# ViTAE-Transformer/MTP

Measured on AMD Instinct MI355X. Metric: images/sec pretrain step (ViT-L+RVSA, 224^2, bf16), higher is better.
Workload: dtype bf16; 1 GPU; ViT-L + RVSA backbone fwd+bwd + grad all-reduce + clip + AdamW, 224x224, batch 64 per GPU (BASELINE configs[2]/[3]); global_batch=64, parallelism=dp1, activation_checkpointing=False, heads=sum_i mean(f_i)

## Files before the change

### mtp_amd/csrc/gemm.hip

```cpp
#include "gemm_common.h"

namespace {

constexpr int BM = 128;
constexpr int BN = 128;
constexpr int NT_THREADS = 256;
constexpr int ROW_BYTES = 128;
constexpr int OPER_BYTES = BM * ROW_BYTES;
constexpr int STAGE_BYTES = 2 * OPER_BYTES;
constexpr int LDS_BYTES = 2 * STAGE_BYTES;

__device__ __forceinline__ int lds_off(int row, int chunk) { return row * ROW_BYTES + ((chunk ^ (row & 7)) << 4); }

__global__ __launch_bounds__(256) void sum_partials_kernel(const float* __restrict__ part, float* __restrict__ out, int64_t n4, int split) {
    for (int64_t i = (int64_t)blockIdx.x * 256 + threadIdx.x; i < n4; i += (int64_t)gridDim.x * 256) {
        float4 s = *reinterpret_cast<const float4*>(part + 4 * i);
        for (int z = 1; z < split; ++z) {
            const float4 v = *reinterpret_cast<const float4*>(part + 4 * (i + (int64_t)z * n4));
            s.x += v.x; s.y += v.y; s.z += v.z; s.w += v.w;
        }
        *reinterpret_cast<float4*>(out + 4 * i) = s;
    }
}

// ... 414 lines not shown
        }
#pragma unroll
        for (int ni = 0; ni < 4; ++ni)
#pragma unroll
            for (int mi = 0; mi < 4; ++mi) Mma<bf16_t>::run(acc[ni][mi], b[ni], a[mi]);
    }
}

__global__ __launch_bounds__(NT_THREADS) __attribute__((amdgpu_waves_per_eu(4, 4))) void gemm_tn_tr_kernel(KArgs p) {
    extern __shared__ __attribute__((aligned(16))) char smem[];
    const int tid = threadIdx.x, lane = tid & 63, wave = __builtin_amdgcn_readfirstlane(tid >> 6);
    const int wm = wave >> 1, wn = wave & 1;
    const int tile = (p.order & 1) ? (int)blockIdx.x : xcd_remap(blockIdx.x, gridDim.x);
    const int tiles_m = (int)gridDim.x / p.tiles_n;
    const int m0 = ((p.order & 2) ? tile % tiles_m : tile / p.tiles_n) * BM, n0 = ((p.order & 2) ? tile / tiles_m : tile % p.tiles_n) * BN;
    const int kt0 = blockIdx.y * p.k_tiles_per_split;
    int kt1 = kt0 + p.k_tiles_per_split;
    kt1 = kt1 < p.k_tiles ? kt1 : p.k_tiles;
    if (kt0 >= kt1) return;
    p.C += (int64_t)blockIdx.y * p.split_stride * (int64_t)sizeof(float);
    f32x4_t acc[4][4];
#pragma unroll
    for (int i = 0; i < 4; ++i)
#pragma unroll
        for (int j = 0; j < 4; ++j) acc[i][j] = f32x4_t{0.f, 0.f, 0.f, 0.f};
    const bool do_colsum = p.colsum != nullptr && n0 == 0;
    float cs[8] = {0.f, 0.f, 0.f, 0.f, 0.f, 0.f, 0.f, 0.f};
    for (int kt = kt0; kt < kt1; ++kt) {
        stage_tn_glds(p, smem, smem + OPER_BYTES, m0, n0, kt, wave, lane);
        asm volatile("s_waitcnt vmcnt(0)" ::: "memory");
        __syncthreads();
        compute_stage_tr(smem, smem + OPER_BYTES, acc, wm, wn, lane);
        if (do_colsum) {
#pragma unroll
            for (int j = 0; j < 4; ++j) {
                const uint4 v = *reinterpret_cast<const uint4*>(smem + ((tid >> 4) + 16 * j) * TR_ROW_BYTES + (tid & 15) * 16);
                const uint32_t w[4] = {v.x, v.y, v.z, v.w};
#pragma unroll
                for (int e = 0; e < 4; ++e) {
                    cs[2 * e] += __uint_as_float(w[e] << 16);
                    cs[2 * e + 1] += __uint_as_float(w[e] & 0xffff0000u);
                }
            }
        }
        __syncthreads();
    }
    if (do_colsum) {
        float* red = reinterpret_cast<float*>(smem);
        const int rg = tid >> 4, f = (rg & 3) | ((rg >> 1) & 4), chunk = (tid & 15) ^ (f << 1);
        *reinterpret_cast<float4*>(red + rg * BM + chunk * 8) = make_float4(cs[0], cs[1], cs[2], cs[3]);
        *reinterpret_cast<float4*>(red + rg * BM + chunk * 8 + 4) = make_float4(cs[4], cs[5], cs[6], cs[7]);
        __syncthreads();
        if (tid < BM) {
            float s = 0.f;
#pragma unroll
            for (int r = 0; r < 16; ++r) s += red[r * BM + tid];
            if (m0 + tid < p.M) atomicAdd(p.colsum + m0 + tid, s);
        }
    }
    epilogue<float, MTP_EPI_BIAS, 4>(p, acc, m0 + wm * 64, n0 + wn * 64, lane);
}

template <typename T>
int fill_common(const mtp_gemm_args* a, KArgs& k) {
    constexpr int E = Elem<T>::kPerChunk;
    if (!a->A || !a->B || !a->C || a->M <= 0 || a->N <= 0 || a->K <= 0) return MTP_ERR_ARG;
    if (a->M > INT32_MAX || a->N > INT32_MAX || a->K > INT32_MAX) return MTP_ERR_ARG;
    if ((a->lda % E) || (a->ldb % E) || (a->ldc % 4) || (a->N % 4)) return MTP_ERR_ARG;
    if (((uintptr_t)a->A | (uintptr_t)a->B | (uintptr_t)a->C) & 15) return MTP_ERR_ARG;
    k.A = (const char*)a->A; k.B = (const char*)a->B; k.C = (char*)a->C;
    k.M = (int)a->M; k.N = (int)a->N; k.K = (int)a->K;
    k.lda = a->lda; k.ldb = a->ldb; k.ldc = a->ldc;
    k.bias = a->bias; k.bias_mod = (int)a->bias_mod;
    k.res = a->res; k.res_ld = a->res_ld; k.res_mod = (int)a->res_mod;
    k.rowscale = a->rowscale; k.rows_per_sample = (int)(a->rows_per_sample > 0 ? a->rows_per_sample : 1);
    k.aux = (char*)a->aux; k.aux_ld = a->aux_ld;
    k.tiles_n = (int)((a->N + BN - 1) / BN);
    k.k_tiles = (int)((a->K + 8 * E - 1) / (8 * E));
    k.k_tiles_per_split = k.k_tiles;
    k.atomic_out = 0;
    k.order = (a->variant >> 1) & 3;
    k.split_stride = 0;
    k.colsum = nullptr;
    return 0;
}

int nt_p8_mode(const mtp_gemm_args* a, const KArgs& k, int cus) {
    if (a->in_dtype != MTP_BF16 || (a->variant & 1024) || !mtp_nt_p8_fits(k, a->out_dtype, a->epilogue)) return 0;
    const int forced = (a->variant >> 8) & 3;
    if (forced) return forced;
    const int64_t tiles = ((a->M + 255) / 256) * ((a->N + 255) / 256) * 256 / cus;
    return (tiles >= 72 || (tiles >= 40 && a->K >= 1536)) ? 1 : 0;
}

int nt_s8_mode(const mtp_gemm_args* a, const KArgs& k, int cus) {
    if (a->in_dtype != MTP_BF16 || (a->variant & (1024 | (1 << 18))) || ((a->variant >> 8) & 3) || !mtp_nt_s8_fits(k, a->out_dtype, a->epilogue)) return 0;
    if (a->variant & (1 << 17)) return 1;
    const int64_t tiles = ((a->M + 255) / 256) * ((a->N + 255) / 256) * 256 / cus;
    return tiles >= 40 && tiles <= 128;
}

template <typename T, typename Tout, int EPI>
int launch_nt(const mtp_gemm_args* a, hipStream_t stream) {
    constexpr int E = Elem<T>::kPerChunk;
    KArgs k;
    int rc = fill_common<T>(a, k);
    if (rc) return rc;
    if (a->K % E) return MTP_ERR_ARG;
    if (EPI == MTP_EPI_BIAS_RES && (!a->res || (a->res_ld % 4))) return MTP_ERR_ARG;
    if ((EPI == MTP_EPI_BIAS_GELU || EPI == MTP_EPI_DGELU || EPI == MTP_EPI_BIAS_GELU_DG || EPI == MTP_EPI_MUL) && (!a->aux || (a->aux_ld % 4))) return MTP_ERR_ARG;
    if (a->bias && a->bias_mod > 0 && (a->bias_mod % 4)) return MTP_ERR_ARG;
    if constexpr (sizeof(T) == 2) {
        const int cus = mtp_stream_cus(stream);
        if (nt_s8_mode(a, k, cus)) return mtp_nt_s8_launch(k, a->out_dtype, EPI, ((((a->variant >> 1) & 3) == 1) ? 2 : 0), stream);
        const int p8 = nt_p8_mode(a, k, cus);
        if (p8) return mtp_nt_p8_launch(k, a->out_dtype, EPI, (p8 == 2 ? 1 : p8 == 3 ? 4 : 0) | ((((a->variant >> 1) & 3) == 1) ? 2 : 0) | (((a->variant >> 15) & 3) << 8) | (((a->variant >> 20) & 3) << 13), stream);
    }
    const int tiles_m = (k.M + BM - 1) / BM;
    dim3 grid(tiles_m * k.tiles_n), block(NT_THREADS);
    const bool glds = ((a->variant & 1) == 0) && (a->K % (8 * E) == 0);
    const int ord = (a->variant >> 1) & 3;
    k.order = ord == 0 ? (k.tiles_n > 8 ? 2 : 0) : ord == 1 ? 1 : ord == 2 ? 2 : 0;
    if (!glds) k.order = ord;
    const int tiles_m8 = (k.M + NT8_BM - 1) / NT8_BM;
    const bool one_round = tiles_m8 * k.tiles_n >= 256 && tiles_m8 * k.tiles_n <= 512;
    if (glds && ((a->variant & 32) || (one_round && !(a->variant & 64)))) {
        if (ord == 0) k.order = k.tiles_n > 8 ? 2 : 0;
        hipLaunchKernelGGL((gemm_nt_sb8_kernel<T, Tout, EPI>), dim3(tiles_m8 * k.tiles_n), dim3(NT8_THREADS), NT8_STAGE_BYTES, stream, k);
        return mtp_launch_status();
    }
    if (glds)
        hipLaunchKernelGGL((gemm_nt_sb_kernel<T, Tout, EPI>), grid, block, STAGE_BYTES, stream, k);
    else
        hipLaunchKernelGGL((gemm_nt_kernel<T, Tout, EPI, false>), grid, block, LDS_BYTES, stream, k);
    return mtp_launch_status();
}

template <typename T>
int launch_tn(const mtp_gemm_args* a, hipStream_t stream) {
    constexpr int E = Elem<T>::kPerChunk;
    KArgs k;
    int rc = fill_common<T>(a, k);
    if (rc) return rc;
    if (a->out_dtype != MTP_F32 || (a->M % E) || (a->N % E)) return MTP_ERR_ARG;
    k.bias = nullptr;
    int split = a->split_k > 1 ? a->split_k : 1;
    if (split > k.k_tiles) split = k.k_tiles;
    k.k_tiles_per_split = (k.k_tiles + split - 1) / split;
    split = (k.k_tiles + k.k_tiles_per_split - 1) / k.k_tiles_per_split;
    const bool use_ws = split > 1 && a->aux != nullptr;
    k.atomic_out = split > 1 && !use_ws;
    k.split_stride = 0;
    if (split > 1) {
        if (a->ldc != a->N) return MTP_ERR_ARG;
        if (use_ws) {
            if ((uintptr_t)a->aux & 15) return MTP_ERR_ARG;
            k.C = (char*)a->aux;
            k.split_stride = (int64_t)a->M * a->N;
        } else {
            hipError_t e = hipMemsetAsync(a->C, 0, sizeof(float) * (size_t)a->M * (size_t)a->N, stream);
            if (e != hipSuccess) return (int)e;
        }
    }
    const int tiles_m = (k.M + BM - 1) / BM;
    dim3 grid(tiles_m * k.tiles_n, split), block(NT_THREADS);
    const bool full = (a->K % (8 * E) == 0) && (a->M % BM == 0) && (a->N % BN == 0);
    const bool tr = sizeof(T) == 2 && !(a->variant & 16) && (full || ((a->K % 64 == 0) && (a->M % 8 == 0) && (a->N % 8 == 0) && a->M >= 8 && a->N >= 8 && !(a->variant & 32768)));
    if (a->colsum && !tr) {
        rc = mtp_colsum_acc(a->A, a->in_dtype, a->lda, a->colsum, a->K, a->M, stream);
        if (rc) return rc;
    }
    if (tr) {
        k.colsum = a->colsum;
        const int ord = (a->variant >> 1) & 3;
        k.order = ord == 0 ? (a->N > a->M ? 2 : 0) : ord == 1 ? 1 : ord == 2 ? 2 : 0;
        hipLaunchKernelGGL(gemm_tn_tr_kernel, grid, block, STAGE_BYTES, stream, k);
    } else if (full && (a->variant & 8))
        hipLaunchKernelGGL((gemm_tn_sb_kernel<T, true>), grid, block, STAGE_BYTES, stream, k);
    else if (full)
        hipLaunchKernelGGL((gemm_tn_kernel<T, true>), grid, block, LDS_BYTES, stream, k);
    else
        hipLaunchKernelGGL((gemm_tn_kernel<T, false>), grid, block, LDS_BYTES, stream, k);
    if (use_ws && !a->defer_sum) {
        const int64_t n4 = (int64_t)a->M * a->N / 4;
        int64_t nb = (n4 + 255) / 256;
        hipLaunchKernelGGL(sum_partials_kernel, dim3((unsigned)(nb > 4096 ? 4096 : nb)), dim3(256), 0, stream, (const float*)a->aux, (float*)a->C, n4, split);
    }
    return mtp_launch_status();
}

struct SumJobs {
    const float* part[MTP_MAX_SEGMENTS];
    float* out[MTP_MAX_SEGMENTS];
    int64_t n4[MTP_MAX_SEGMENTS];
    int split[MTP_MAX_SEGMENTS];
};
__global__ __launch_bounds__(256) void sum_partials_batch_kernel(SumJobs t) {
    const int j = blockIdx.y;
    const float* __restrict__ part = t.part[j];
// ... 73 lines not shown
```

### mtp_amd/csrc/gemm_common.h

```cpp
#pragma once
#include "common.h"

struct KArgs {
    const char* A;
    const char* B;
    char* C;
    int M, N, K;
    int64_t lda, ldb, ldc;
    const float* bias;
    int bias_mod;
    const float* res;
    int64_t res_ld;
    int res_mod;
    const float* rowscale;
    int rows_per_sample;
    char* aux;
    int64_t aux_ld;
    int tiles_n;
    int k_tiles;
    int k_tiles_per_split;
    int atomic_out;
    int order;
    int64_t split_stride;
    float* colsum;
};

int mtp_nt_p8_launch(const KArgs& k, int out_dtype, int epilogue, int flags, hipStream_t stream);
int mtp_nt_p8_fits(const KArgs& k, int out_dtype, int epilogue);
int mtp_nt_s8_launch(const KArgs& k, int out_dtype, int epilogue, int flags, hipStream_t stream);
int mtp_nt_s8_fits(const KArgs& k, int out_dtype, int epilogue);

namespace {

template <typename T>
struct Mma;
template <>
struct Mma<bf16_t> {
    __device__ static __forceinline__ void run(f32x4_t& acc, const uint4& a, const uint4& b) {
        acc = __builtin_amdgcn_mfma_f32_16x16x32_bf16(__builtin_bit_cast(bf16x8_t, a), __builtin_bit_cast(bf16x8_t, b), acc, 0, 0, 0);
    }
};
template <>
struct Mma<float> {
    __device__ static __forceinline__ void run(f32x4_t& acc, const uint4& a, const uint4& b) {
        acc = __builtin_amdgcn_mfma_f32_16x16x4f32(__uint_as_float(a.x), __uint_as_float(b.x), acc, 0, 0, 0);
        acc = __builtin_amdgcn_mfma_f32_16x16x4f32(__uint_as_float(a.y), __uint_as_float(b.y), acc, 0, 0, 0);
        acc = __builtin_amdgcn_mfma_f32_16x16x4f32(__uint_as_float(a.z), __uint_as_float(b.z), acc, 0, 0, 0);
        acc = __builtin_amdgcn_mfma_f32_16x16x4f32(__uint_as_float(a.w), __uint_as_float(b.w), acc, 0, 0, 0);
    }
};

__device__ __attribute__((aligned(16))) const uint4 g_zero16 = {0u, 0u, 0u, 0u};

__device__ __forceinline__ int xcd_remap(int bid, int nb) {
    int xcd = bid & 7, idx = bid >> 3, q = nb >> 3, r = nb & 7;
    return (xcd < r ? xcd * (q + 1) : r * (q + 1) + (xcd - r) * q) + idx;
}


template <typename Tout, int EPI, int MF>
__device__ __forceinline__ void epilogue(const KArgs& p, f32x4_t (&acc)[4][MF], int mrow0, int ncol0, int lane) {
    const int fr = lane & 15, g = lane >> 4;
    Tout* C = reinterpret_cast<Tout*>(p.C);
    int nn[4];
    bool nok[4];
    float4 bias[4];
#pragma unroll
    for (int ni = 0; ni < 4; ++ni) {
        const int n = ncol0 + ni * 16 + g * 4;
        nok[ni] = n < p.N;
        nn[ni] = nok[ni] ? n : 0;
        const float* bp = (EPI != MTP_EPI_DGELU && EPI != MTP_EPI_MUL && p.bias) ? p.bias + (p.bias_mod > 0 ? nn[ni] % p.bias_mod : nn[ni]) : reinterpret_cast<const float*>(&g_zero16);
        const uint4 b = ldg16(bp);
        bias[ni] = make_float4(__uint_as_float(b.x), __uint_as_float(b.y), __uint_as_float(b.z), __uint_as_float(b.w));
    }
#pragma unroll
    for (int mi = 0; mi < MF; ++mi) {
        const int m = mrow0 + mi * 16 + fr;
        const bool mok = m < p.M;
        const int mc = mok ? m : 0;
        if (p.atomic_out) {
#pragma unroll
            for (int ni = 0; ni < 4; ++ni)
                if (mok && nok[ni]) {
                    float* c = reinterpret_cast<float*>(p.C) + (int64_t)m * p.ldc + nn[ni];
                    atomicAdd(c + 0, acc[ni][mi][0]); atomicAdd(c + 1, acc[ni][mi][1]); atomicAdd(c + 2, acc[ni][mi][2]); atomicAdd(c + 3, acc[ni][mi][3]);
                }
            continue;
        }
        float rs = 1.0f;
        float4 side[4];
        if (EPI == MTP_EPI_BIAS_RES) {
            const float* rsp = p.rowscale ? p.rowscale + mc / p.rows_per_sample : nullptr;
            const float* resrow = p.res + (int64_t)(p.res_mod > 0 ? mc % p.res_mod : mc) * p.res_ld;
#pragma unroll
            for (int ni = 0; ni < 4; ++ni) {
                const uint4 r = ldg16(resrow + nn[ni]);
                side[ni] = make_float4(__uint_as_float(r.x), __uint_as_float(r.y), __uint_as_float(r.z), __uint_as_float(r.w));
            }
            if (rsp) rs = *rsp;
        } else if (EPI == MTP_EPI_DGELU || EPI == MTP_EPI_MUL) {
#pragma unroll
            for (int ni = 0; ni < 4; ++ni) side[ni] = load4(reinterpret_cast<const Tout*>(p.aux) + (int64_t)mc * p.aux_ld + nn[ni]);
        }
#pragma unroll
        for (int ni = 0; ni < 4; ++ni) {
            float4 v = make_float4(acc[ni][mi][0] + bias[ni].x, acc[ni][mi][1] + bias[ni].y, acc[ni][mi][2] + bias[ni].z, acc[ni][mi][3] + bias[ni].w);
// ... 22 lines not shown
```

### mtp_amd/csrc/gemm_p8.hip

```cpp
#include "gemm_p8.h"

namespace {

struct P8Ctx {
    uint32_t addrA[2][2];
    uint32_t addrA1[2][2];
    uint32_t addrB[2][2];
    uint32_t voffA, voffB;
    const char* pA[2][2];
    const char* pB[2][2];
    uint32_t m0base;
};

template <int IMM>
__device__ __forceinline__ void dsr(u32x4_t& d, uint32_t addr) {
    asm volatile("ds_read_b128 %0, %1 offset:%2" : "=v"(d) : "v"(addr), "i"(IMM));
}

template <int SK, int SBUF>
__device__ __forceinline__ void nt_stage(const P8Ctx& c) {
    constexpr int h = (SK == KA1 || SK == KB1) ? 1 : 0;
    const uint32_t l0 = c.m0base + SBUF * P8_BUF + SK * P8_HALF;
    if constexpr (SK == KA0 || SK == KA1)
        glds2(c.voffA, c.pA[h][0], c.pA[h][1], l0, l0 + 1024);
    else
        glds2(c.voffB, c.pB[h][0], c.pB[h][1], l0, l0 + 1024);
}

template <int K, int BUF, int MI>
__device__ __forceinline__ void nt_read_a(const P8Ctx& c, u32x4_t (&a)[2][4]) {
    constexpr int o = K * P8_HALF;
    const uint32_t a0 = K == KA1 ? c.addrA1[BUF][0] : c.addrA[BUF][0], a1 = K == KA1 ? c.addrA1[BUF][1] : c.addrA[BUF][1];
    dsr<o + 0 * 2048>(a[0][0], a0); dsr<o + 1 * 2048>(a[0][1], a0); dsr<o + 2 * 2048>(a[0][2], a0);
    if constexpr (MI == 4) dsr<o + 3 * 2048>(a[0][3], a0);
    dsr<o + 0 * 2048>(a[1][0], a1); dsr<o + 1 * 2048>(a[1][1], a1); dsr<o + 2 * 2048>(a[1][2], a1);
    if constexpr (MI == 4) dsr<o + 3 * 2048>(a[1][3], a1);
}
template <int K, int BUF>
__device__ __forceinline__ void nt_read_b(const P8Ctx& c, u32x4_t (&b)[2][2]) {
    constexpr int o = K * P8_HALF;
    dsr<o + 0 * 2048>(b[0][0], c.addrB[BUF][0]); dsr<o + 1 * 2048>(b[0][1], c.addrB[BUF][0]);
    dsr<o + 0 * 2048>(b[1][0], c.addrB[BUF][1]); dsr<o + 1 * 2048>(b[1][1], c.addrB[BUF][1]);
}
template <int MI>
__device__ __forceinline__ void wait_a(u32x4_t (&a)[2][4]) {
    if constexpr (MI == 4)
        asm volatile("s_waitcnt lgkmcnt(0)"
                     : "+v"(a[0][0]), "+v"(a[0][1]), "+v"(a[0][2]), "+v"(a[0][3]), "+v"(a[1][0]), "+v"(a[1][1]), "+v"(a[1][2]), "+v"(a[1][3]));
    else
        asm volatile("s_waitcnt lgkmcnt(0)" : "+v"(a[0][0]), "+v"(a[0][1]), "+v"(a[0][2]), "+v"(a[1][0]), "+v"(a[1][1]), "+v"(a[1][2]));
}
__device__ __forceinline__ void wait_b(u32x4_t (&b)[2][2]) {
    asm volatile("s_waitcnt lgkmcnt(0)" : "+v"(b[0][0]), "+v"(b[0][1]), "+v"(b[1][0]), "+v"(b[1][1]));
}

template <int MI1>
struct NtOps {
    typedef P8Ctx Ctx;
    static constexpr int kLoadsPerPiecePair = 2;
    static constexpr int kMi1 = MI1;
    template <int K, int BUF> static __device__ __forceinline__ void read_a(Ctx& c, u32x4_t (&a)[2][4]) { nt_read_a<K, BUF, (K == KA1 ? MI1 : 4)>(c, a); }
    template <int K, int BUF> static __device__ __forceinline__ void read_b(Ctx& c, u32x4_t (&b)[2][2]) { nt_read_b<K, BUF>(c, b); }
    template <int SK, int SBUF> static __device__ __forceinline__ void stage(Ctx& c) { nt_stage<SK, SBUF>(c); }
    template <int K, int BUF> static __device__ __forceinline__ void retire_a(Ctx&, u32x4_t (&a)[2][4]) { wait_a<(K == KA1 ? MI1 : 4)>(a); }
    static __device__ __forceinline__ void retire_b(u32x4_t (&b)[2][2]) { wait_b(b); }
    static __device__ __forceinline__ void next_ktile(Ctx& c) { c.voffA += 128; c.voffB += 128; }
};

template <int MI1>
__device__ __forceinline__ void p8_tile_sources(const KArgs& p, P8Ctx& c, int wave, int m0, int n0, uint32_t voffA0, uint32_t voffB0) {
    constexpr int WROWS = 64 + 16 * MI1;
#pragma unroll
    for (int i = 0; i < 2; ++i) {
        const int q = wave * 2 + i;
        int ra0 = m0 + (q >> 3) * WROWS + (q & 7) * 8;
        const int qw = q / (2 * MI1), qx = q - qw * (2 * MI1);
        int ra1 = qw < 2 ? m0 + qw * WROWS + 64 + qx * 8 : m0;
        ra0 = ra0 < p.M - 8 ? ra0 : p.M - 8;
        ra1 = ra1 < p.M - 8 ? ra1 : p.M - 8;
        c.pA[0][i] = p.A + (int64_t)ra0 * p.lda * 2;
        c.pA[1][i] = p.A + (int64_t)ra1 * p.lda * 2;
#pragma unroll
        for (int h = 0; h < 2; ++h) {
            int rb = n0 + (q >> 2) * 64 + h * 32 + (q & 3) * 8;
            rb = rb < p.N - 8 ? rb : p.N - 8;
            c.pB[h][i] = p.B + (int64_t)rb * p.ldb * 2;
        }
    }
    c.voffA = voffA0;
    c.voffB = voffB0;
}
__device__ __forceinline__ void p8_issue_prologue(P8Ctx& c) {
    nt_stage<KB1, 0>(c); nt_stage<KA0, 0>(c); nt_stage<KB0, 0>(c); nt_stage<KA1, 0>(c);
    c.voffA += 128; c.voffB += 128;
    nt_stage<KB0, 1>(c); nt_stage<KA0, 1>(c); nt_stage<KB1, 1>(c); nt_stage<KA1, 1>(c);
    c.voffA += 128; c.voffB += 128;
}

template <typename Tout, int EPI, int MI1, int XP, int PS, int SP = 0>
__global__ __launch_bounds__(P8_THREADS) __attribute__((amdgpu_waves_per_eu(2, 2))) void gemm_nt_p8_kernel(KArgs p) {
    extern __shared__ __attribute__((aligned(16))) char smem[];
    constexpr int WROWS = 64 + 16 * MI1, BM = 2 * WROWS;
    const int tid = threadIdx.x, lane = tid & 63;
    const int wave = __builtin_amdgcn_readfirstlane(tid >> 6);
    const int wr = wave >> 2, wc = wave & 3;
    const int fr = lane & 15, g = lane >> 4;
    const uint32_t lds0 = (uint32_t)(uintptr_t)(__attribute__((address_space(3))) char*)(smem);
    const int tiles_m = (p.M + BM - 1) / BM, tiles_n = p.tiles_n, ntiles = tiles_m * tiles_n;
    const int plain = p.order & 1;
    const int pairs = p.k_tiles >> 1;

    P8Ctx c;
    {
        const uint32_t lanepart = (uint32_t)(fr * 128 + ((g ^ (fr & 7)) << 4));
#pragma unroll
        for (int b = 0; b < 2; ++b) {
            c.addrA[b][0] = lds0 + b * P8_BUF + wr * 8192 + lanepart;
            c.addrA[b][1] = lds0 + b * P8_BUF + wr * 8192 + (lanepart ^ 64u);
            c.addrA1[b][0] = lds0 + b * P8_BUF + wr * (MI1 * 2048) + lanepart;
            c.addrA1[b][1] = lds0 + b * P8_BUF + wr * (MI1 * 2048) + (lanepart ^ 64u);
            c.addrB[b][0] = lds0 + b * P8_BUF + wc * 4096 + lanepart;
            c.addrB[b][1] = lds0 + b * P8_BUF + wc * 4096 + (lanepart ^ 64u);
        }
        c.m0base = lds0 + wave * 2048;
    }
    const uint32_t lanesrc = (uint32_t)(((lane & 7) ^ (lane >> 3)) << 4);
    const uint32_t voffA0 = (uint32_t)((lane >> 3) * (int)p.lda * 2) + lanesrc;
    const uint32_t voffB0 = (uint32_t)((lane >> 3) * (int)p.ldb * 2) + lanesrc;

    int tile = blockIdx.x;
    int tm, tn;
    tile_coords(plain ? tile : xcd_remap(tile, ntiles), tiles_m, tiles_n, plain, tm, tn);
    int m0 = tm * BM, n0 = tn * P8_BN;
    p8_tile_sources<MI1>(p, c, wave, m0, n0, voffA0, voffB0);
    p8_issue_prologue(c);

    u32x4_t a[2][4], b0[2][2], b1[2][2];
    f32x4_t acc[4][8];
    for (;;) {
#pragma unroll
        for (int i = 0; i < 4; ++i)
#pragma unroll
            for (int j = 0; j < 8; ++j) acc[i][j] = f32x4_t{0.f, 0.f, 0.f, 0.f};

        wait_vm<12>();
        __builtin_amdgcn_sched_barrier(0);
        __builtin_amdgcn_s_barrier();
        __builtin_amdgcn_sched_barrier(0);
        nt_read_b<KB1, 0>(c, b1);
        wait_b(b1);
        __builtin_amdgcn_sched_barrier(0);
        __builtin_amdgcn_s_barrier();
        if (!(XP & 2) && wr == 1) __builtin_amdgcn_s_barrier();
        __builtin_amdgcn_sched_barrier(0);

        for (int it = 0; it < pairs - 1; ++it) two_tiles<NtOps<MI1>, false, XP>(c, a, b0, b1, acc);
        two_tiles<NtOps<MI1>, true, XP>(c, a, b0, b1, acc);

        __builtin_amdgcn_sched_barrier(0);
        if (!(XP & 2) && wr == 0) __builtin_amdgcn_s_barrier();
        __builtin_amdgcn_sched_barrier(0);

        if constexpr (PS) {
            const int em0 = m0, en0 = n0;
            tile += gridDim.x;
            const bool more = tile < ntiles;
            if (more) {
                tile_coords(plain ? tile : xcd_remap(tile, ntiles), tiles_m, tiles_n, plain, tm, tn);
                m0 = tm * BM; n0 = tn * P8_BN;
                p8_tile_sources<MI1>(p, c, wave, m0, n0, voffA0, voffB0);
                p8_issue_prologue(c);
            }
            __builtin_amdgcn_sched_barrier(0);
            epilogue_lds16<Tout, EPI, WROWS, SP>(p, acc, smem + P8_LDS + wave * 4096, em0 + wr * WROWS, en0 + wc * 64, lane);
            if (!more) break;
            __builtin_amdgcn_sched_barrier(0);
            wait_vm<0>();
        } else {
            if constexpr (SP != 0) {
                epilogue_lds16<Tout, EPI, WROWS, SP>(p, acc, smem + P8_LDS + wave * 4096, m0 + wr * WROWS, n0 + wc * 64, lane);
            } else if (!(XP & 4) || p.M < 0) {
                if constexpr (XP & 16)
                    epilogue<Tout, EPI, 8>(p, acc, m0 + wr * 128, n0 + wc * 64, lane);
                else
                    epilogue_lds<Tout, EPI, 64, 32, WROWS>(p, acc, smem + wave * P8_HALF, m0 + wr * WROWS, n0 + wc * 64, lane);
            }
            break;
        }
    }
}

template <typename Tout, int EPI, int MI1, int XP, int PS = 0, int SP = 0>
int launch_p8_kernel(const KArgs& a, int ntiles, hipStream_t stream) {
    constexpr int LDS = P8_LDS + ((PS || SP) ? 8 * 4096 : 0);
    static unsigned long long optin = 0;
    if (const int e = mtp_optin_lds((const void*)gemm_nt_p8_kernel<Tout, EPI, MI1, XP, PS, SP>, LDS, optin)) return e;
    const int cus = mtp_stream_cus(stream);
    const int grid = PS ? (ntiles < cus ? ntiles : cus) : ntiles;
    hipLaunchKernelGGL((gemm_nt_p8_kernel<Tout, EPI, MI1, XP, PS, SP>), dim3(grid), dim3(P8_THREADS), LDS, stream, a);
    return mtp_launch_status();
}

int p8_pick_bm(int64_t M, int64_t N, int64_t cus) {
    const int64_t tn = (N + P8_BN - 1) / P8_BN;
    const int64_t t256 = ((M + 255) / 256) * tn, t224 = ((M + 223) / 224) * tn;
    const int64_t c256 = ((t256 + cus - 1) / cus) * 256, c224 = ((t224 + cus - 1) / cus) * 224;
    return c224 < c256 ? 224 : 256;
}

template <typename Tout, int EPI>
int launch_p8(const KArgs& k, int flags, hipStream_t stream) {
    const int bm = (flags & 1) ? 224 : (flags & 4) ? 256 : p8_pick_bm(k.M, k.N, mtp_stream_cus(stream));
    const int tiles_m = (k.M + bm - 1) / bm, tiles_n = (k.N + P8_BN - 1) / P8_BN;
    KArgs a = k;
    a.tiles_n = tiles_n;
    a.k_tiles = k.K / 64;
    a.order = (flags >> 1) & 1;
    a.atomic_out = 0;
    const int ntiles = tiles_m * tiles_n;
    const bool persist = (flags & 256) || (!(flags & 512) && bm == 224 && ntiles > mtp_stream_cus(stream));
    int sp = (flags >> 13) & 3;
    if (sp == 0) sp = (EPI == MTP_EPI_BIAS_RES) ? 2 : 1;
    if (bm == 224 && sp == 1) return persist ? launch_p8_kernel<Tout, EPI, 3, 0, 1, 1>(a, ntiles, stream) : launch_p8_kernel<Tout, EPI, 3, 0, 0, 1>(a, ntiles, stream);
    if (bm == 224 && sp == 2) return persist ? launch_p8_kernel<Tout, EPI, 3, 0, 1, 2>(a, ntiles, stream) : launch_p8_kernel<Tout, EPI, 3, 0, 0, 2>(a, ntiles, stream);
    if (persist) {
        if (bm == 224) return launch_p8_kernel<Tout, EPI, 3, 0, 1>(a, ntiles, stream);
        return launch_p8_kernel<Tout, EPI, 4, 0, 1>(a, ntiles, stream);
    }
    if (bm == 224) return launch_p8_kernel<Tout, EPI, 3, 0>(a, ntiles, stream);
    return launch_p8_kernel<Tout, EPI, 4, 0>(a, ntiles, stream);
}

template <typename Tout>
int dispatch_p8(const KArgs& k, int epi, int flags, hipStream_t s) {
    switch (epi) {
        case MTP_EPI_BIAS: return launch_p8<Tout, MTP_EPI_BIAS>(k, flags, s);
        case MTP_EPI_BIAS_GELU: return launch_p8<Tout, MTP_EPI_BIAS_GELU>(k, flags, s);
        case MTP_EPI_DGELU: return launch_p8<Tout, MTP_EPI_DGELU>(k, flags, s);
        case MTP_EPI_BIAS_GELU_DG: return launch_p8<Tout, MTP_EPI_BIAS_GELU_DG>(k, flags, s);
        case MTP_EPI_MUL: return launch_p8<Tout, MTP_EPI_MUL>(k, flags, s);
        default: return MTP_ERR_UNSUPPORTED;
    }
}

}

int mtp_nt_p8_fits(const KArgs& k, int out_dtype, int epi) {
    if (k.K < 128 || (k.K % 128) || (k.M % 8) || (k.N % 8) || k.M < 8 || k.N < 8) return 0;
    if ((uint64_t)k.lda * 2 * 8 + (uint64_t)k.K * 2 >= (1ull << 31) || (uint64_t)k.ldb * 2 * 8 + (uint64_t)k.K * 2 >= (1ull << 31)) return 0;
    if (epi == MTP_EPI_BIAS_RES) return out_dtype == MTP_F32;
    if (out_dtype == MTP_BF16) return epi == MTP_EPI_BIAS || epi == MTP_EPI_BIAS_GELU || epi == MTP_EPI_DGELU || epi == MTP_EPI_BIAS_GELU_DG || epi == MTP_EPI_MUL;
    return out_dtype == MTP_F32 && epi == MTP_EPI_BIAS;
}

int mtp_nt_p8_launch(const KArgs& k, int out_dtype, int epi, int flags, hipStream_t stream) {
    if (!mtp_nt_p8_fits(k, out_dtype, epi)) return MTP_ERR_UNSUPPORTED;
    if (epi == MTP_EPI_BIAS_RES) return launch_p8<float, MTP_EPI_BIAS_RES>(k, flags, stream);
    if (out_dtype == MTP_BF16) return dispatch_p8<bf16_t>(k, epi, flags, stream);
    return launch_p8<float, MTP_EPI_BIAS>(k, flags, stream);
}
```

### mtp_amd/engine.py

```python
import os

import torch

from . import ops

F32 = torch.float32


class _Blk:
    __slots__ = ("window", "pre", "wqkv", "wqkvT", "wproj", "wprojT", "w1", "w1T", "w2", "w2T", "wsamp", "bsamp", "bproj", "b2", "wproj_s", "w2_s")


class BackboneEngine:
    def __init__(self, module, act_dtype=torch.bfloat16):
        self.m = module
        self.act = act_dtype
        self.C = module.embed_dim
        self.depth = len(module.blocks)
        self.heads = module.num_heads
        self.hd = self.C // self.heads
        self.scale = module.qk_scale if module.qk_scale is not None else self.hd ** -0.5
        self.window = [bool(w) for w in module.window_blocks]
        self.out_indices = list(module.out_indices)
        self._key = None
        self._ln_parts = []
        self._sl_jobs = []
        self._blk = None
        self._fpn = None
        self._pe = None
        self._wimg = None
        self._wimg_ptrs = None
        self._ls = []
        self._zero_rel = {}

    def params(self):
        return dict(self.m.named_parameters())

    def _weights_key(self, P):
        return (self.act,) + tuple((p.data_ptr(), p._version) for p in P.values())

    def prepare_weights(self, force=False):
        P = self.params()
        key = self._weights_key(P)
        if not force and key == self._key:
            return
        ptrs = (self.act,) + tuple(p.data_ptr() for p in P.values())
        if self._wimg is None or ptrs != self._wimg_ptrs:
            self._build_weight_images(P)
            self._wimg_ptrs = ptrs
        with torch.no_grad():
            for pre, b in self._ls:
                g1, g2 = P[pre + "gamma_1"].detach(), P[pre + "gamma_2"].detach()
                torch.mul(P[pre + "attn.proj.weight"].detach(), g1[:, None], out=b.wproj_s)
                torch.mul(P[pre + "mlp.fc2.weight"].detach(), g2[:, None], out=b.w2_s)
                torch.mul(P[pre + "attn.proj.bias"].detach(), g1, out=b.bproj)
                torch.mul(P[pre + "mlp.fc2.bias"].detach(), g2, out=b.b2)
        if force or getattr(self, "_images_fresh", None) != key:
            self._wimg.refresh()
        self._images_fresh = None
        for name, (wg, wgT) in self._fpn.items():
            ops.convt_pack(P[name + ".weight"].detach().contiguous(), wg, wgT)
        self._key = key

    def mark_images_fresh(self):
        self._images_fresh = self._weights_key(self.params())
        self._key = None

    def _build_weight_images(self, P):
        dev = P["patch_embed.proj.weight"].device
        act, H, C = self.act, self.heads, self.C
        entries = []

        def both(w2d):
            w2d = w2d.detach()
            assert w2d.is_contiguous()
            R, Cc = w2d.shape
            wt = torch.empty(Cc, R, device=dev, dtype=act)
            w = w2d if act == F32 else torch.empty(R, Cc, device=dev, dtype=act)
            entries.append((w2d, None if act == F32 else w, wt, False))
            return w, wt

        ls = getattr(self.m, "init_values", None) is not None
        self._ls = []

        blks = []
        for i in range(self.depth):
            b = _Blk()
            b.window = self.window[i]
            b.pre = pre = "blocks.%d." % i
# ... 63 lines not shown
        return ops.colsum(dy, out, accumulate=True)

    def _ln_bwd(self, *args, **kw):
        return ops.layernorm_bwd(*args, accumulate=True, defer=self._ln_parts, **kw)

    def _ln_flush(self):
        if self._ln_parts:
            ops.reduce_rows_deferred(self._ln_parts)
        if self._sl_jobs:
            ops.small_linear_dw_segments_flush(self._sl_jobs)

    def _full_rel(self, pre, Hp, Wp):
        h = self.P.get(pre + "attn.full_attn_rel_pos_h")
        if h is not None:
            w = self.P[pre + "attn.full_attn_rel_pos_w"]
            if h.shape[0] < 2 * Hp - 1 or w.shape[0] < 2 * Wp - 1:
                raise ValueError("%sattn.full_attn_rel_pos_h/w have %d / %d rows, a %d x %d token grid needs %d / %d (resize them like "
                                 "init_weights does, or build the model for this input size)" % (pre, h.shape[0], w.shape[0], Hp, Wp, 2 * Hp - 1, 2 * Wp - 1))
            return h[:2 * Hp - 1], w[:2 * Wp - 1]
        key = (Hp, Wp)
        if self._zero_rel.get(key) is None:
            self._zero_rel[key] = (torch.zeros(2 * Hp - 1, self.hd, device=self.dev, dtype=F32),
                                   torch.zeros(2 * Wp - 1, self.hd, device=self.dev, dtype=F32))
        return self._zero_rel[key]

    def _drop_scales(self, B, training):
        rates = [float(self.m.drop_path_rates[i]) for i in range(self.depth)]
        live = [training and r > 0.0 and self.m.blocks[i].training for i, r in enumerate(rates)]
        if not any(live):
            return [(None, None)] * self.depth
        keep = torch.tensor([1.0 - r for r in rates], dtype=F32).to(self.dev, non_blocking=True).view(self.depth, 1, 1)
        s = torch.floor(keep + torch.rand(self.depth, 2, B, device=self.dev, dtype=F32)) / keep
        return [(s[i, 0], s[i, 1]) if live[i] else (None, None) for i in range(self.depth)]

    def _block_fwd(self, i, x, B, Hp, Wp, dps, save):
        P, b, C, T, N = self.P, self._blk[i], self.C, x.shape[0], Hp * Wp
        pre = b.pre
        s = {}
        mean1, rstd1 = self._e(T, dtype=F32), self._e(T, dtype=F32)
        ln1 = ops.layernorm_fwd(x, P[pre + "norm1.weight"], P[pre + "norm1.bias"], self._e(T, C), mean1, rstd1)
        if b.window:
            nh, nw = ops.rvsa_windows(Hp, Wp)
            R = B * nh * nw
            avg, pooled = self._e(R, C, dtype=F32), self._e(R, C, dtype=F32)
            samp = ops.rvsa_sampling_fwd(ln1, b.wsamp, b.bsamp, avg, pooled, self._e(R, 5 * self.heads, dtype=F32), B, Hp, Wp)
        qkv = ops.gemm_nt(ln1, b.wqkv, self._e(T, 3 * C), bias=P[pre + "attn.qkv.bias"])
        o = self._e(T, C)
        if b.window:
            lse = self._e(R * self.heads * 49, dtype=F32)
            ops.rvsa_attn_fwd(qkv, samp, o, lse, P[pre + "attn.rel_pos_h"], P[pre + "attn.rel_pos_w"],
                              P[pre + "attn.relative_position_bias_table"], B, Hp, Wp, self.heads, self.scale)
            s.update(avg=avg, pooled=pooled, samp=samp)
        else:
            lse = self._e(B * self.heads * N, dtype=F32)
            rel_h, rel_w = self._full_rel(pre, Hp, Wp)
            ops.full_attn_fwd(qkv, o, lse, rel_h, rel_w, B, Hp, Wp, self.heads, self.scale)
        x1 = ops.gemm_nt(o, b.wproj, self._e(T, C, dtype=F32), epi=ops.EPI_BIAS_RES, bias=b.bproj, res=x,
                         rowscale=dps[0], rows_per_sample=N)
        mean2, rstd2 = self._e(T, dtype=F32), self._e(T, dtype=F32)
        ln2 = ops.layernorm_fwd(x1, P[pre + "norm2.weight"], P[pre + "norm2.bias"], self._e(T, C), mean2, rstd2)
        u = self._e(T, 4 * C)
        h = ops.gemm_nt(ln2, b.w1, self._e(T, 4 * C), epi=ops.EPI_BIAS_GELU_DG, bias=P[pre + "mlp.fc1.bias"], aux=u)
        x2 = ops.gemm_nt(h, b.w2, self._e(T, C, dtype=F32), epi=ops.EPI_BIAS_RES, bias=b.b2, res=x1,
                         rowscale=dps[1], rows_per_sample=N)
        if save:
            s.update(x=x, mean1=mean1, rstd1=rstd1, ln1=ln1, qkv=qkv, o=o, lse=lse, x1=x1, mean2=mean2, rstd2=rstd2, ln2=ln2, u=u, h=h)
        return x2, s

    def _layer_scale_grads(self, pre, lin, gname, G):
        P = self.P
        gw, gb, gam = G[pre + lin + ".weight"], G[pre + lin + ".bias"], P[pre + gname]
        G[pre + gname].add_((gw * P[pre + lin + ".weight"]).sum(1) + gb * P[pre + lin + ".bias"])
        gw.mul_(gam[:, None])
        gb.mul_(gam)

    def _block_bwd(self, i, s, dx2, dx2_act, B, Hp, Wp, dps, G, extra, prev_scale):
        P, b, C, N = self.P, self._blk[i], self.C, Hp * Wp
        pre = b.pre
        T = dx2.shape[0]
        wq = self._wq
        ls = pre + "gamma_1" in G
        wq.add(dx2_act, s["h"], G[pre + "mlp.fc2.weight"], G[pre + "mlp.fc2.bias"], after=(lambda: self._layer_scale_grads(pre, "mlp.fc2", "gamma_2", G)) if ls else None,
               norm_ok=not ls)
        du = ops.gemm_nt(dx2_act, b.w2T, self._e(T, 4 * C), epi=ops.EPI_MUL, aux=s["u"])
        wq.add(du, s["ln2"], G[pre + "mlp.fc1.weight"], G[pre + "mlp.fc1.bias"])
        dln2 = ops.gemm_nt(du, b.w1T, self._e(T, C))
        del du
        dx1, dx1_act = self._e(T, C, dtype=F32), self._e(T, C)
        self._ln_bwd(dln2, s["x1"], s["mean2"], s["rstd2"], P[pre + "norm2.weight"], dx1, G[pre + "norm2.weight"], G[pre + "norm2.bias"],
                          dres=dx2, dx_copy=dx1_act, copy_scale=dps[0], rows_per_sample=N)
        wq.add(dx1_act, s["o"], G[pre + "attn.proj.weight"], G[pre + "attn.proj.bias"], after=(lambda: self._layer_scale_grads(pre, "attn.proj", "gamma_1", G)) if ls else None,
               norm_ok=not ls)
        do = ops.gemm_nt(dx1_act, b.wprojT, self._e(T, C))
        dqkv = self._e(T, 3 * C)
        if b.window:
            nh, nw = ops.rvsa_windows(Hp, Wp)
            R = B * nh * nw
            H = self.heads
            dsamp = self._e(R, 5 * H, dtype=F32)
            ops.rvsa_attn_bwd(s["qkv"], s["samp"], s["o"], do, s["lse"], dqkv, dsamp,
                              P[pre + "attn.rel_pos_h"], P[pre + "attn.rel_pos_w"], P[pre + "attn.relative_position_bias_table"],
                              G[pre + "attn.rel_pos_h"], G[pre + "attn.rel_pos_w"], G[pre + "attn.relative_position_bias_table"],
                              B, Hp, Wp, H, self.scale, accumulate=True, defer=self._ln_parts)
            names = ("sampling_offsets", "sampling_scales", "sampling_angles")
            self._sl_jobs.append((s["pooled"], dsamp, [G[pre + "attn.%s.2.weight" % n].view(-1, C) for n in names],
                                  [G[pre + "attn.%s.2.bias" % n] for n in names]))
        else:
            rel_h, rel_w = self._full_rel(pre, Hp, Wp)
            if pre + "attn.full_attn_rel_pos_h" in G:
                drel_h, drel_w = G[pre + "attn.full_attn_rel_pos_h"][:2 * Hp - 1], G[pre + "attn.full_attn_rel_pos_w"][:2 * Wp - 1]
            else:
                drel_h, drel_w = self._e(*rel_h.shape, dtype=F32), self._e(*rel_w.shape, dtype=F32)
            ops.full_attn_bwd(s["qkv"], s["o"], do, s["lse"], dqkv, rel_h, rel_w, drel_h, drel_w, B, Hp, Wp, self.heads, self.scale,
                              accumulate=True, defer=self._ln_parts)
        wq.add(dqkv, s["ln1"], G[pre + "attn.qkv.weight"], G[pre + "attn.qkv.bias"])
        win_add = None
        if b.window:
            win_add = ops.rvsa_sampling_bwd_win(dsamp, b.wsamp, s["avg"], self._e(*s["avg"].shape, dtype=F32))
        dln1 = ops.gemm_nt(dqkv, b.wqkvT, self._e(T, C))
        dx0, dx0_act = self._e(T, C, dtype=F32), self._e(T, C)
        self._ln_bwd(dln1, s["x"], s["mean1"], s["rstd1"], P[pre + "norm1.weight"], dx0, G[pre + "norm1.weight"], G[pre + "norm1.bias"],
                          dres=dx1, extra=extra, dx_copy=dx0_act, copy_scale=prev_scale, rows_per_sample=N,
                          **(dict(win_add=win_add, grid=(B, Hp, Wp)) if win_add is not None else {}))
        return dx0, dx0_act

    def forward(self, img, training=False, need_grad=False, feature_dtype=None):
        m = self.m
        self.dev = img.device
        self.prepare_weights()
        self.P = P = {k: v.detach() for k, v in self.params().items()}
        C, act = self.C, self.act
        ps = m.patch_size
        fdt = feature_dtype or act
        if img.dtype == torch.uint8:
            pp = getattr(m, "data_preprocessor", None)
            if pp is None:
                raise ValueError("uint8 input needs ViT_Win_RVSA_V3_WSZ7.set_data_preprocessor(mean, std, ...)")
            B, H, W, Cin = img.shape
            Hp, Wp = ops.padded_grid(H, W, ps, pp["pad_size_divisor"])
            N, T = Hp * Wp, B * Hp * Wp
            cols = ops.preprocess_patchify(img.contiguous(), self._e(T, Cin * ps * ps), ps, pp["mean"], pp["std"], pp["bgr_to_rgb"],
                                           pp["pad_size_divisor"], pp["pad_value"])
            H, W = Hp * ps, Wp * ps
        else:
            B, Cin, H, W = img.shape
            Hp, Wp = H // ps, W // ps
            N, T = Hp * Wp, B * Hp * Wp
            img = img.contiguous()
            if img.dtype != F32:
                img = img.float()
            cols = ops.patchify(img, self._e(T, Cin * ps * ps), ps)
        pos = P.get("pos_embed")
        if pos is not None:
            assert pos.shape[1] == N, "pos_embed does not match the input size"
            x = ops.gemm_nt(cols, self._pe[0], self._e(T, C, dtype=F32), epi=ops.EPI_BIAS_RES, bias=P["patch_embed.proj.bias"],
                            res=pos.reshape(N, C), res_mod=N)
        else:
            x = ops.gemm_nt(cols, self._pe[0], self._e(T, C, dtype=F32), bias=P["patch_embed.proj.bias"])
        dps = self._drop_scales(B, training)
        ckpt = bool(m.use_checkpoint) and need_grad
        saved, taps = [], {}
        vitdet = bool(getattr(m, "_vitdet", False))
        last = self.depth - 1 if vitdet else max(self.out_indices)
        for i in range(self.depth):
            if i > last:
                break
            xin = x
# ... 10 lines not shown
        else:
            tap_list = [taps[i] for i in self.out_indices]
        if getattr(m, "_taps_only", False):
            feats = [ops.tokens_to_nchw(t, self._e(B, C, Hp, Wp, dtype=fdt), B, Hp, Wp, 0) for t in tap_list]
            fctx = {"taps_only": True}
        else:
            feats, fctx = self._fpn_fwd(tap_list, B, Hp, Wp, fdt, need_grad)
        ctx = None
        if need_grad:
            ctx = dict(saved=saved, dps=dps, fctx=fctx, cols=cols, geom=(B, Cin, H, W, Hp, Wp), ckpt=ckpt, last=last, final=final)
        return feats, ctx

    def _fpn_fwd(self, taps, B, Hp, Wp, fdt, need_grad):
        P, C, T = self.P, self.C, B * Hp * Wp
        m = self.m
        feats, fctx = [], {}
        if m.patch_size == 8:
            t0 = taps[0] if self.act == F32 else ops.cast(taps[0], self._e(T, C))
            z = ops.gemm_nt(t0, self._fpn["fpn1.0"][0], self._e(T, 4 * C), bias=P["fpn1.0.bias"], bias_mod=C)
            feats.append(ops.tokens_to_nchw(z.view(4 * T, C), self._e(B, C, 2 * Hp, 2 * Wp, dtype=fdt), B, Hp, Wp, 1))
            feats.append(ops.tokens_to_nchw(taps[1], self._e(B, C, Hp, Wp, dtype=fdt), B, Hp, Wp, 0))
            H2, W2, H4, W4 = Hp // 2, Wp // 2, Hp // 4, Wp // 4
            p3 = ops.maxpool2_tokens_fwd(taps[2], self._e(B * H2 * W2, C), B, Hp, Wp)
            feats.append(ops.tokens_to_nchw(p3, self._e(B, C, H2, W2, dtype=fdt), B, H2, W2, 0))
            q1 = ops.maxpool2_tokens_fwd(taps[3], self._e(B * H2 * W2, C, dtype=F32), B, Hp, Wp)
            q2 = ops.maxpool2_tokens_fwd(q1, self._e(B * H4 * W4, C), B, H2, W2)
            feats.append(ops.tokens_to_nchw(q2, self._e(B, C, H4, W4, dtype=fdt), B, H4, W4, 0))
            if need_grad:
                fctx = dict(p8=True, t0=t0, tap2=taps[2], tap3=taps[3], q1=q1)
            return feats, fctx
        if m.patch_size != 16:
            raise NotImplementedError("the reference defines the FPN tail for patch_size 16 and 8 only (VIT:640-670)")
        t0 = taps[0] if self.act == F32 else ops.cast(taps[0], self._e(T, C))
        y1 = ops.gemm_nt(t0, self._fpn["fpn1.0"][0], self._e(T, 4 * C), bias=P["fpn1.0.bias"], bias_mod=C)
        mean, rstd = self._e(4 * T, dtype=F32), self._e(4 * T, dtype=F32)
        g1 = ops.layernorm_fwd(y1.view(4 * T, C), P["fpn1.1.ln.weight"], P["fpn1.1.ln.bias"], self._e(4 * T, C), mean, rstd, gelu=True)
        y2 = ops.gemm_nt(g1, self._fpn["fpn1.3"][0], self._e(4 * T, 4 * C), bias=P["fpn1.3.bias"], bias_mod=C)
        feats.append(ops.tokens_to_nchw(y2.view(16 * T, C), self._e(B, C, 4 * Hp, 4 * Wp, dtype=fdt), B, Hp, Wp, 2))
        t1 = taps[1] if self.act == F32 else ops.cast(taps[1], self._e(T, C))
        z = ops.gemm_nt(t1, self._fpn["fpn2.0"][0], self._e(T, 4 * C), bias=P["fpn2.0.bias"], bias_mod=C)
        feats.append(ops.tokens_to_nchw(z.view(4 * T, C), self._e(B, C, 2 * Hp, 2 * Wp, dtype=fdt), B, Hp, Wp, 1))
        feats.append(ops.tokens_to_nchw(taps[2], self._e(B, C, Hp, Wp, dtype=fdt), B, Hp, Wp, 0))
        Ho, Wo = Hp // 2, Wp // 2
        pooled = ops.maxpool2_tokens_fwd(taps[3], self._e(B * Ho * Wo, C), B, Hp, Wp)
        feats.append(ops.tokens_to_nchw(pooled, self._e(B, C, Ho, Wo, dtype=fdt), B, Ho, Wo, 0))
        if need_grad:
            fctx = dict(t0=t0, y1=y1, mean=mean, rstd=rstd, g1=g1, t1=t1, tap3=taps[3])
        return feats, fctx

    def _convt_wgrad(self, dy, x, gw):
        dwg = self._e(dy.shape[1], x.shape[1], dtype=F32)
        self._wq.add(dy, x, dwg, after=lambda: ops.convt_unpack_grad(dwg, gw), norm_of=gw)

    def _fpn_bwd(self, dfeats, fctx, B, Hp, Wp, G):
        P, C, T, act = self.P, self.C, B * Hp * Wp, self.act
        out = [None] * 4

        def as_in(df):
            df = df.contiguous()
            return df if df.dtype in (F32, torch.bfloat16) else df.float()

        if fctx.get("p8"):
            H2, W2, H4, W4 = Hp // 2, Wp // 2, Hp // 4, Wp // 4
            if dfeats[0] is not None:
                dz = ops.nchw_to_tokens(as_in(dfeats[0]), self._e(4 * T, C), B, Hp, Wp, 1)
                self._convt_wgrad(dz.view(T, 4 * C), fctx["t0"], G["fpn1.0.weight"])
                self._colsum(dz, G["fpn1.0.bias"])
                out[0] = ops.gemm_nt(dz.view(T, 4 * C), self._fpn["fpn1.0"][1], self._e(T, C, dtype=F32))
            if dfeats[1] is not None:
                out[1] = ops.nchw_to_tokens(as_in(dfeats[1]), self._e(T, C, dtype=F32), B, Hp, Wp, 0)
            if dfeats[2] is not None:
                dp = ops.nchw_to_tokens(as_in(dfeats[2]), self._e(B * H2 * W2, C, dtype=F32), B, H2, W2, 0)
                out[2] = ops.maxpool2_tokens_bwd(fctx["tap2"], dp, self._e(T, C, dtype=F32), B, Hp, Wp)
            if dfeats[3] is not None:
                dq2 = ops.nchw_to_tokens(as_in(dfeats[3]), self._e(B * H4 * W4, C, dtype=F32), B, H4, W4, 0)
                dq1 = ops.maxpool2_tokens_bwd(fctx["q1"], dq2, self._e(B * H2 * W2, C, dtype=F32), B, H2, W2)
                out[3] = ops.maxpool2_tokens_bwd(fctx["tap3"], dq1, self._e(T, C, dtype=F32), B, Hp, Wp)
            return out

        if dfeats[0] is not None:
            dy2 = ops.nchw_to_tokens(as_in(dfeats[0]), self._e(16 * T, C), B, Hp, Wp, 2)
            self._convt_wgrad(dy2.view(4 * T, 4 * C), fctx["g1"], G["fpn1.3.weight"])
            self._colsum(dy2, G["fpn1.3.bias"])
            dg1 = ops.gemm_nt(dy2.view(4 * T, 4 * C), self._fpn["fpn1.3"][1], self._e(4 * T, C))
            dy1 = self._e(4 * T, C)
            self._ln_bwd(dg1, fctx["y1"].view(4 * T, C), fctx["mean"], fctx["rstd"], P["fpn1.1.ln.weight"], dy1,
                              G["fpn1.1.ln.weight"], G["fpn1.1.ln.bias"], beta=P["fpn1.1.ln.bias"], gelu=True)
            self._convt_wgrad(dy1.view(T, 4 * C), fctx["t0"], G["fpn1.0.weight"])
            self._colsum(dy1, G["fpn1.0.bias"])
            out[0] = ops.gemm_nt(dy1.view(T, 4 * C), self._fpn["fpn1.0"][1], self._e(T, C, dtype=F32))
        if dfeats[1] is not None:
            dz = ops.nchw_to_tokens(as_in(dfeats[1]), self._e(4 * T, C), B, Hp, Wp, 1)
            self._convt_wgrad(dz.view(T, 4 * C), fctx["t1"], G["fpn2.0.weight"])
            self._colsum(dz, G["fpn2.0.bias"])
            out[1] = ops.gemm_nt(dz.view(T, 4 * C), self._fpn["fpn2.0"][1], self._e(T, C, dtype=F32))
        if dfeats[2] is not None:
            out[2] = ops.nchw_to_tokens(as_in(dfeats[2]), self._e(T, C, dtype=F32), B, Hp, Wp, 0)
        if dfeats[3] is not None:
            Ho, Wo = Hp // 2, Wp // 2
            dp = ops.nchw_to_tokens(as_in(dfeats[3]), self._e(B * Ho * Wo, C, dtype=F32), B, Ho, Wo, 0)
            out[3] = ops.maxpool2_tokens_bwd(fctx["tap3"], dp, self._e(T, C, dtype=F32), B, Hp, Wp)
        return out

    def backward(self, ctx, dfeats, G, need_input_grad=False, on_block_done=None, split_last=False, sqn=None):
        B, Cin, H, W, Hp, Wp = ctx["geom"]
        C, N, T = self.C, Hp * Wp, B * Hp * Wp
        P = self.P
        self.dev = ctx["cols"].device
        self._ln_parts = []
        self._sl_jobs = []
        self._wq = wq = ops.WgradQueue(stream=self._wgrad_stream())
        wq.max_jobs = self.wgrad_max_jobs if wq.stream is not None else 0
        wq.sqn = sqn
        self.norm_covered = wq.covered
        if ctx["fctx"].get("taps_only"):
            dtaps = [None if d is None else ops.nchw_to_tokens((d.contiguous() if d.dtype in (F32, torch.bfloat16) else d.float().contiguous()),
                                                               self._e(T, C, dtype=F32), B, Hp, Wp, 0) for d in dfeats]
        else:
            dtaps = self._fpn_bwd(dfeats, ctx["fctx"], B, Hp, Wp, G)
        tapgrad = {}
        last, dps, saved = ctx["last"], ctx["dps"], ctx["saved"]
        if ctx.get("final") is not None:
            dsum = None
            for d in dtaps:
                if d is None:
                    continue
                if dsum is None:
                    dsum = d
                else:
                    ops.axpy(dsum, d)
            if dsum is not None:
                xl, fm, fr = ctx["final"]
                tapgrad[last] = self._ln_bwd(dsum, xl, fm, fr, P["norm.weight"], self._e(T, C, dtype=F32), G["norm.weight"], G["norm.bias"])
        else:
            for idx, d in zip(self.out_indices, dtaps):
                if d is None:
                    continue
                if idx in tapgrad:
                    ops.axpy(tapgrad[idx], d)
                else:
                    tapgrad[idx] = d
        self._ln_flush()
        if on_block_done is not None and not wq.jobs:
            on_block_done(self.depth)
        if last not in tapgrad:
            tapgrad[last] = torch.zeros(T, C, device=self.dev, dtype=F32)
        dx = tapgrad[last]
        dx_act = self._scaled_copy(dx, dps[last][1], N)
        waiting = []
        pending = []
        for i in range(last, -1, -1):
            s = saved[i]
            if ctx["ckpt"]:
                _, s = self._block_fwd(i, s["x"], B, Hp, Wp, dps[i], save=True)
            extra = tapgrad.get(i - 1) if i > 0 else None
            prev_scale = dps[i - 1][1] if i > 0 else None
            dx, dx_act = self._block_bwd(i, s, dx, dx_act, B, Hp, Wp, dps[i], G, extra, prev_scale)
            saved[i] = None
            waiting.append(i)
            if i == 0:
                wq.add(dx_act, ctx["cols"], G["patch_embed.proj.weight"].view(C, -1), G["patch_embed.proj.bias"])
            if i == 0 or wq.should_flush() or not wq.jobs or (split_last and i == 1):
                wq.flush()
                self._ln_flush()
                if wq.stream is None:
                    if on_block_done is not None:
                        on_block_done(waiting[-1])
# ... 24 lines not shown
```

Measured before the change: 1894 images/sec.

## Stagger persistent p8 GEMM blocks and use grouped tile order for tail balance

```diff
diff --git a/mtp_amd/csrc/gemm.hip b/mtp_amd/csrc/gemm.hip
--- a/mtp_amd/csrc/gemm.hip
+++ b/mtp_amd/csrc/gemm.hip
@@ -520,6 +520,8 @@
     k.order = (a->variant >> 1) & 3;
     k.split_stride = 0;
     k.colsum = nullptr;
+    k.stagger_from = 0;
+    k.stagger_ticks = 0;
     return 0;
 }
 
@@ -552,7 +554,7 @@
         const int cus = mtp_stream_cus(stream);
         if (nt_s8_mode(a, k, cus)) return mtp_nt_s8_launch(k, a->out_dtype, EPI, ((((a->variant >> 1) & 3) == 1) ? 2 : 0), stream);
         const int p8 = nt_p8_mode(a, k, cus);
-        if (p8) return mtp_nt_p8_launch(k, a->out_dtype, EPI, (p8 == 2 ? 1 : p8 == 3 ? 4 : 0) | ((((a->variant >> 1) & 3) == 1) ? 2 : 0) | (((a->variant >> 15) & 3) << 8) | (((a->variant >> 20) & 3) << 13), stream);
+        if (p8) return mtp_nt_p8_launch(k, a->out_dtype, EPI, (p8 == 2 ? 1 : p8 == 3 ? 4 : 0) | ((((a->variant >> 1) & 3) == 1) ? 2 : 0) | (((a->variant >> 15) & 3) << 8) | (((a->variant >> 20) & 3) << 13) | (((a->variant >> 22) & 15) << 16), stream);
     }
     const int tiles_m = (k.M + BM - 1) / BM;
     dim3 grid(tiles_m * k.tiles_n), block(NT_THREADS);
diff --git a/mtp_amd/csrc/gemm_common.h b/mtp_amd/csrc/gemm_common.h
--- a/mtp_amd/csrc/gemm_common.h
+++ b/mtp_amd/csrc/gemm_common.h
@@ -23,6 +23,8 @@
     int order;
     int64_t split_stride;
     float* colsum;
+    int stagger_from;
+    int stagger_ticks;
 };
 
 int mtp_nt_p8_launch(const KArgs& k, int out_dtype, int epilogue, int flags, hipStream_t stream);
diff --git a/mtp_amd/csrc/gemm_p8.hip b/mtp_amd/csrc/gemm_p8.hip
--- a/mtp_amd/csrc/gemm_p8.hip
+++ b/mtp_amd/csrc/gemm_p8.hip
@@ -1,3 +1,6 @@
+#include <atomic>
+#include <cstdlib>
+
 #include "gemm_p8.h"
 
 namespace {
@@ -97,6 +100,17 @@
     c.voffA += 128; c.voffB += 128;
 }
 
+__device__ __forceinline__ void p8_coords(int t, int tiles_m, int tiles_n, int order, int& tm, int& tn) {
+    const int per = 8 * tiles_n, grp = t / per, r = t - grp * per;
+    if ((order & 5) == 4 && tiles_m - grp * 8 >= 8 && (tiles_n & 3) == 0) {
+        const int b16 = r >> 4, j = r & 15;
+        tm = grp * 8 + (b16 & 1) * 4 + (j & 3);
+        tn = (b16 >> 1) * 4 + (j >> 2);
+        return;
+    }
+    tile_coords(t, tiles_m, tiles_n, order & 1, tm, tn);
+}
+
 template <typename Tout, int EPI, int MI1, int XP, int PS, int SP = 0>
 __global__ __launch_bounds__(P8_THREADS) __attribute__((amdgpu_waves_per_eu(2, 2))) void gemm_nt_p8_kernel(KArgs p) {
     extern __shared__ __attribute__((aligned(16))) char smem[];
@@ -128,9 +142,15 @@
     const uint32_t voffA0 = (uint32_t)((lane >> 3) * (int)p.lda * 2) + lanesrc;
     const uint32_t voffB0 = (uint32_t)((lane >> 3) * (int)p.ldb * 2) + lanesrc;
 
+    if constexpr (PS) {
+        if (p.stagger_ticks > 0 && (int)blockIdx.x >= p.stagger_from) {
+            const uint64_t until = wall_clock64() + (uint64_t)p.stagger_ticks;
+            while (wall_clock64() < until) __builtin_amdgcn_s_sleep(8);
+        }
+    }
     int tile = blockIdx.x;
     int tm, tn;
-    tile_coords(plain ? tile : xcd_remap(tile, ntiles), tiles_m, tiles_n, plain, tm, tn);
+    p8_coords(plain ? tile : xcd_remap(tile, ntiles), tiles_m, tiles_n, p.order, tm, tn);
     int m0 = tm * BM, n0 = tn * P8_BN;
     p8_tile_sources<MI1>(p, c, wave, m0, n0, voffA0, voffB0);
     p8_issue_prologue(c);
@@ -166,7 +186,7 @@
             tile += gridDim.x;
             const bool more = tile < ntiles;
             if (more) {
-                tile_coords(plain ? tile : xcd_remap(tile, ntiles), tiles_m, tiles_n, plain, tm, tn);
+                p8_coords(plain ? tile : xcd_remap(tile, ntiles), tiles_m, tiles_n, p.order, tm, tn);
                 m0 = tm * BM; n0 = tn * P8_BN;
                 p8_tile_sources<MI1>(p, c, wave, m0, n0, voffA0, voffB0);
                 p8_issue_prologue(c);
@@ -190,6 +210,25 @@
     }
 }
 
+int p8_ticks_per_us() {
+    static std::atomic<int> rate[64];
+    int dev = 0;
+    if (hipGetDevice(&dev) != hipSuccess || dev < 0 || dev >= 64) return 100;
+    int r = rate[dev].load(std::memory_order_relaxed);
+    if (!r) {
+        int khz = 0;
+        if (hipDeviceGetAttribute(&khz, hipDeviceAttributeWallClockRate, dev) != hipSuccess || khz < 1000) khz = 100000;
+        r = khz / 1000;
+        rate[dev].store(r, std::memory_order_relaxed);
+    }
+    return r;
+}
+
+int p8_stagger_env() {
+    static const int v = []() { const char* e = getenv("MTP_NT_STAGGER"); return e && (e[0] == '0' || e[0] == '1') ? e[0] - '0' : -1; }();
+    return v;
+}
+
 template <typename Tout, int EPI, int MI1, int XP, int PS = 0, int SP = 0>
 int launch_p8_kernel(const KArgs& a, int ntiles, hipStream_t stream) {
     constexpr int LDS = P8_LDS + ((PS || SP) ? 8 * 4096 : 0);
@@ -219,6 +258,19 @@
     a.atomic_out = 0;
     const int ntiles = tiles_m * tiles_n;
     const bool persist = (flags & 256) || (!(flags & 512) && bm == 224 && ntiles > mtp_stream_cus(stream));
+    a.stagger_from = 0;
+    a.stagger_ticks = 0;
+    if (persist) {
+        const int cus = mtp_stream_cus(stream), grid = ntiles < cus ? ntiles : cus, rem = ntiles % grid;
+        const int env = p8_stagger_env();
+        const bool on = env >= 0 ? env == 1 : (flags & (1 << 16)) ? true : (flags & (1 << 17)) ? false : true;
+        if (on && rem) {
+            const int q = ((flags >> 18) & 3) ? ((flags >> 18) & 3) : 2;
+            a.stagger_from = rem;
+            a.stagger_ticks = (int)((int64_t)q * a.k_tiles * 1030 * p8_ticks_per_us() / 4000);
+            a.order |= 4;
+        }
+    }
     int sp = (flags >> 13) & 3;
     if (sp == 0) sp = (EPI == MTP_EPI_BIAS_RES) ? 2 : 1;
     if (bm == 224 && sp == 1) return persist ? launch_p8_kernel<Tout, EPI, 3, 0, 1, 1>(a, ntiles, stream) : launch_p8_kernel<Tout, EPI, 3, 0, 0, 1>(a, ntiles, stream);
diff --git a/mtp_amd/engine.py b/mtp_amd/engine.py
--- a/mtp_amd/engine.py
+++ b/mtp_amd/engine.py
@@ -5,6 +5,7 @@
 from . import ops
 
 F32 = torch.float32
+BWD_NT_VARIANT = 0
 
 
 class _Blk:
@@ -234,7 +235,7 @@
         ls = pre + "gamma_1" in G
         wq.add(dx2_act, s["h"], G[pre + "mlp.fc2.weight"], G[pre + "mlp.fc2.bias"], after=(lambda: self._layer_scale_grads(pre, "mlp.fc2", "gamma_2", G)) if ls else None,
                norm_ok=not ls)
-        du = ops.gemm_nt(dx2_act, b.w2T, self._e(T, 4 * C), epi=ops.EPI_MUL, aux=s["u"])
+        du = ops.gemm_nt(dx2_act, b.w2T, self._e(T, 4 * C), epi=ops.EPI_MUL, aux=s["u"], variant=BWD_NT_VARIANT)
         wq.add(du, s["ln2"], G[pre + "mlp.fc1.weight"], G[pre + "mlp.fc1.bias"])
         dln2 = ops.gemm_nt(du, b.w1T, self._e(T, C))
         del du
@@ -411,7 +412,7 @@
             dy2 = ops.nchw_to_tokens(as_in(dfeats[0]), self._e(16 * T, C), B, Hp, Wp, 2)
             self._convt_wgrad(dy2.view(4 * T, 4 * C), fctx["g1"], G["fpn1.3.weight"])
             self._colsum(dy2, G["fpn1.3.bias"])
-            dg1 = ops.gemm_nt(dy2.view(4 * T, 4 * C), self._fpn["fpn1.3"][1], self._e(4 * T, C))
+            dg1 = ops.gemm_nt(dy2.view(4 * T, 4 * C), self._fpn["fpn1.3"][1], self._e(4 * T, C), variant=BWD_NT_VARIANT)
             dy1 = self._e(4 * T, C)
             self._ln_bwd(dg1, fctx["y1"].view(4 * T, C), fctx["mean"], fctx["rstd"], P["fpn1.1.ln.weight"], dy1,
                               G["fpn1.1.ln.weight"], G["fpn1.1.ln.bias"], beta=P["fpn1.1.ln.bias"], gelu=True)
```

After: 1919 images/sec, median of 6. +1.3%, better.
